# shizukutanaka/Otedama

Hardware: AMD Instinct MI355X
Metric: hashes/sec (whole node) SHA-256d + scrypt at 1/2/4/8 MI355X; p50 share latency (higher is better)
Workload: dtype u32

## Files before the change

### csrc/bindings.cpp

```cpp
#include <pybind11/pybind11.h>
#include <pybind11/stl.h>

#include <array>
#include <atomic>
#include <cstring>
#include <stdexcept>
#include <thread>
#include <tuple>

#include "otedama/aead.h"
#include "otedama/job.h"
#include "otedama/runtime.h"
#include "otedama/trace.h"
#include "otedama/sha256.h"
#include "otedama/sv2_frame.h"
#include "otedama/clock_bounds.h"
#include "otedama/launch_plan.h"
#include "otedama/search_launch.h"
#include "otedama/share_job.h"
#include "otedama/work_queue.h"
#include "otedama/x11.h"

namespace py = pybind11;
using namespace otedama;
// ... 314 lines not shown
  }, py::arg("header"), py::arg("target"), py::arg("start"), py::arg("count"));
  m.def("cpu_scan_method", &cpu_scan_method);
  m.def("_cpu_scan_lanes", [](int lanes, const py::bytes& h, const py::bytes& t, uint32_t start, uint64_t count) {
    std::string hs = need(h, 80, "header"), ts = need(t, 32, "target");
    std::vector<uint32_t> hits;
    {
      py::gil_scoped_release r;
      hits = cpu_scan_sha256d_lanes(lanes, reinterpret_cast<const uint8_t*>(hs.data()),
                                    reinterpret_cast<const uint8_t*>(ts.data()), start, count);
    }
    return hits;
  });
  m.def("merkle_root", [](const py::dict& job, uint64_t en2) {
    auto j = make_job(job); uint8_t root[32];
    merkle_root_from_coinbase(*j, en2, root);
    return to_bytes(root, 32);
  });
  m.def("variant_header", [](const py::dict& job, uint64_t v) {
    auto j = make_job(job);
    uint8_t hdr[80]; uint32_t ver, nt; uint64_t en2;
    j->variant_header(v, hdr, &ver, &nt, &en2);
    return py::make_tuple(to_bytes(hdr, 80), ver, nt, en2);
  });
  m.def("variant_space", [](const py::dict& job) { return make_job(job)->variant_space(); });

  m.def("sha256d_prepare", [](const py::bytes& h, const py::bytes& t) {
    std::string hs = need(h, 80, "header"), ts = need(t, 32, "target");
    Sha256dParams p;
    sha256d_prepare(reinterpret_cast<const uint8_t*>(hs.data()), reinterpret_cast<const uint8_t*>(ts.data()), &p);
    return py::bytes(reinterpret_cast<const char*>(&p), sizeof p);
  });
  m.attr("SHA256D_MAX_K") = kSha256dMaxK;
  {
    py::list ks;
    for (int k = 2; k <= kSha256dMaxK; ++k)
      if (sha256d_k_floor(k) == k) ks.append(k);
    m.attr("SHA256D_K_VALUES") = py::tuple(ks);
  }
  m.def("sha256d_prepare_k", [](const py::list& headers, const py::bytes& t) {
    std::string ts = need(t, 32, "target");
    std::vector<std::string> hs;
    for (auto& h : headers) hs.push_back(need(h.cast<py::bytes>(), 80, "header"));
    std::vector<const uint8_t*> ptrs;
    for (auto& h : hs) ptrs.push_back(reinterpret_cast<const uint8_t*>(h.data()));
    Sha256dParamsK p;
    if (!sha256d_prepare_k(ptrs.data(), (int)ptrs.size(), reinterpret_cast<const uint8_t*>(ts.data()), &p))
      throw std::invalid_argument("need K headers (K in SHA256D_K_VALUES) with identical bytes 64..75");
    return py::bytes(reinterpret_cast<const char*>(&p), sizeof p);
  }, py::arg("headers"), py::arg("target"));
  m.attr("SHA256D_V_GROUP") = kSha256dVGroup;
  m.attr("SHA256D_V2_GROUP") = kSha256dV2Group;
  m.def("sha256d_prepare_v", [](const py::list& headers, const py::bytes& t) {
    std::string ts = need(t, 32, "target");
    std::vector<std::string> hs;
    for (auto& h : headers) hs.push_back(need(h.cast<py::bytes>(), 80, "header"));
    std::vector<const uint8_t*> ptrs;
    for (auto& h : hs) ptrs.push_back(reinterpret_cast<const uint8_t*>(h.data()));
    Sha256dParamsV p;
    std::vector<Sha256dVariant> vars(hs.size());
    if (!sha256d_prepare_v(ptrs.data(), (int)ptrs.size(), reinterpret_cast<const uint8_t*>(ts.data()), &p, vars.data()))
      throw std::invalid_argument("need a positive multiple of 64 headers with identical bytes 64..75");
    return py::make_tuple(py::bytes(reinterpret_cast<const char*>(&p), sizeof p),
                          py::bytes(reinterpret_cast<const char*>(vars.data()), vars.size() * sizeof(Sha256dVariant)));
  }, py::arg("headers"), py::arg("target"));
  m.def("scrypt_prepare", [](const py::bytes& h, const py::bytes& t) {
    std::string hs = need(h, 80, "header"), ts = need(t, 32, "target");
    ScryptParams p;
    scrypt_prepare(reinterpret_cast<const uint8_t*>(hs.data()), reinterpret_cast<const uint8_t*>(ts.data()), &p);
    return py::bytes(reinterpret_cast<const char*>(&p), sizeof p);
  });

  m.def("x11_prepare", [](const py::bytes& h, const py::bytes& t) {
    std::string hs = need(h, 80, "header"), ts = need(t, 32, "target");
    X11Params p;
    x11_prepare(reinterpret_cast<const uint8_t*>(hs.data()), reinterpret_cast<const uint8_t*>(ts.data()), &p);
    return py::bytes(reinterpret_cast<const char*>(&p), sizeof p);
  });

  m.def("trace_push", [](const std::string& name) { trace_push(name.c_str()); });
  m.def("trace_pop", [] { trace_pop(); });
  m.def("trace_mark", [](const std::string& name) { trace_mark(name.c_str()); });
  m.def("gpu_device_count", &gpu_device_count);
  m.def("gpu_arch_name", &gpu_arch_name);
  m.def("gpu_cu_count", &gpu_cu_count);
  m.def("scrypt_scratch_bytes", &scrypt_scratch_bytes);
  m.def("x11_midstage_polls", [] { return x11k::x11_midstage_polls(); });
  m.def("_scrypt_romix_mode", [] {
    bool write_polls = false;
    uint32_t segments = 0;
    scrypt_romix_mode(&write_polls, &segments);
    py::dict d;
    d["write_polls"] = write_polls;
    d["segments"] = segments;
    return d;
  });
  m.def("maps_range_writable", [](const std::string& maps, uint64_t lo, uint64_t hi) {
    return maps_range_writable(maps, uintptr_t(lo), uintptr_t(hi));
  });
  m.def("launch_sha256d", [](const py::bytes& params, uint32_t base, uint64_t count, uintptr_t out, uint32_t cap,
                             int grid, uintptr_t stream) {
    std::string ps = need(params, sizeof(Sha256dParams), "params");
    Sha256dParams p; std::memcpy(&p, ps.data(), sizeof p);
    if (count == 0 || count > (1ull << 32)) throw std::invalid_argument("count must be in [1, 2^32]");
    if (grid <= 0 || out == 0) throw std::invalid_argument("bad grid / out");
    py_launch_sha256d(p, base, count, out, cap, grid, stream);
  }, py::arg("params"), py::arg("base"), py::arg("count"), py::arg("out"), py::arg("cap"), py::arg("grid"),
     py::arg("stream"));
  m.def("launch_sha256d_k", [](const py::bytes& params, uint32_t base, uint64_t count, uintptr_t out, uint32_t cap,
                               int grid, uintptr_t stream) {
    std::string ps = need(params, sizeof(Sha256dParamsK), "params");
    Sha256dParamsK p; std::memcpy(&p, ps.data(), sizeof p);
    if (p.k < 2 || p.k > kSha256dMaxK) throw std::invalid_argument("bad K");
    if (count == 0 || count > (1ull << 32)) throw std::invalid_argument("count must be in [1, 2^32]");
    if (grid <= 0 || out == 0) throw std::invalid_argument("bad grid / out");
    py_launch_sha256d_k(p, base, count, out, cap, grid, stream);
  }, py::arg("params"), py::arg("base"), py::arg("count"), py::arg("out"), py::arg("cap"), py::arg("grid"),
     py::arg("stream"));
  m.def("launch_sha256d_v", [](const py::bytes& params, uintptr_t vars, uint32_t base, uint64_t count, uintptr_t out,
                               uint32_t cap, int grid, uintptr_t stream, bool occupancy8, int block, int chains) {
    std::string ps = need(params, sizeof(Sha256dParamsV), "params");
    Sha256dParamsV p; std::memcpy(&p, ps.data(), sizeof p);
    p.occupancy8 = occupancy8 ? 1u : 0u;
    if (p.groups == 0 || count == 0 || count > (1ull << 32)) throw std::invalid_argument("bad groups / count");
    if (block != 64 && block != 256) throw std::invalid_argument("block must be 64 or 256 threads");
    if (chains < 1 || chains > 4) throw std::invalid_argument("chains must be 1..4");
    if (p.groups % uint32_t(chains) != 0)
      throw std::invalid_argument("chains variants per lane need a multiple of 64 * chains variants");
    if (grid <= 0 || (uint64_t(grid) * uint32_t(block / 64)) % (p.groups / uint32_t(chains)) != 0 || vars == 0 || out == 0)
      throw std::invalid_argument("the wave count must be a multiple of the variant groups; vars/out must be set");
    py_launch_sha256d_v(p, vars, base, count, out, cap, grid, stream, block, chains);
  }, py::arg("params"), py::arg("vars"), py::arg("base"), py::arg("count"), py::arg("out"), py::arg("cap"),
     py::arg("grid"), py::arg("stream"), py::arg("occupancy8") = false, py::arg("block") = 256, py::arg("chains") = 1);
  m.def("launch_scrypt", [](const py::bytes& params, uint32_t base, uint32_t count, uintptr_t xbuf, uintptr_t scratch,
                            int gap, uintptr_t out, uint32_t cap, int grid, uintptr_t stream) {
    std::string ps = need(params, sizeof(ScryptParams), "params");
    ScryptParams p; std::memcpy(&p, ps.data(), sizeof p);
    if (!scrypt_gap_valid(gap))
      throw std::invalid_argument("gap must be 1, 2, 4, SCRYPT_COOP or SCRYPT_LANE_W8");
    if (grid <= 0 || out == 0 || xbuf == 0 || scratch == 0 || count == 0) throw std::invalid_argument("bad launch args");
    py_launch_scrypt(p, base, count, xbuf, scratch, gap, out, cap, grid, stream);
  }, py::arg("params"), py::arg("base"), py::arg("count"), py::arg("xbuf"), py::arg("scratch"), py::arg("gap"),
     py::arg("out"), py::arg("cap"), py::arg("grid"), py::arg("stream"));

  m.def("launch_x11_stage", [](const py::bytes& params, int stage, uint32_t base, uintptr_t H, uint32_t stride,
                               uint32_t n, uintptr_t out, uint32_t cap, uintptr_t stream) {
    std::string ps = need(params, sizeof(X11Params), "params");
    X11Params p; std::memcpy(&p, ps.data(), sizeof p);
    if (stage < 0 || stage >= kX11StageCount) throw std::invalid_argument("stage must be in [0, 11)");
    if (H == 0 || n == 0 || stride < n) throw std::invalid_argument("need H != 0, n > 0, stride >= n");
    py_launch_x11_stage(p, stage, base, H, stride, n, out, cap, stream);
  }, py::arg("params"), py::arg("stage"), py::arg("base"), py::arg("H"), py::arg("stride"), py::arg("n"),
     py::arg("out") = 0, py::arg("cap") = 0, py::arg("stream") = 0);
  m.def("launch_x11", [](const py::bytes& params, uint32_t base, uintptr_t H, uint32_t stride, uint32_t n,
                         uintptr_t out, uint32_t cap, uintptr_t stream) {
    std::string ps = need(params, sizeof(X11Params), "params");
    X11Params p; std::memcpy(&p, ps.data(), sizeof p);
    if (H == 0 || n == 0 || stride < n) throw std::invalid_argument("need H != 0, n > 0, stride >= n");
    py_launch_x11(p, base, H, stride, n, out, cap, stream);
  }, py::arg("params"), py::arg("base"), py::arg("H"), py::arg("stride"), py::arg("n"), py::arg("out") = 0,
     py::arg("cap") = 0, py::arg("stream") = 0);

  m.def("launch_sha256d_digest", [](uintptr_t headers, uint32_t n, uintptr_t out, uintptr_t stream) {
    if (headers == 0 || out == 0 || n == 0) throw std::invalid_argument("need headers != 0, out != 0, n > 0");
    py_launch_sha256d_digest(headers, n, out, stream);
  }, py::arg("headers"), py::arg("n"), py::arg("out"), py::arg("stream") = 0);
  m.def("launch_scrypt_digest", [](uintptr_t headers, uint32_t n, uintptr_t xbuf, uintptr_t scratch, int gap,
                                   uintptr_t out, int grid, uintptr_t stream) {
    if (headers == 0 || out == 0 || xbuf == 0 || scratch == 0 || n == 0 || grid <= 0)
      throw std::invalid_argument("bad launch args");
    if (uint64_t(n) > uint64_t(grid) * 256u) throw std::invalid_argument("n must be at most grid * 256");
    py_launch_scrypt_digest(headers, n, xbuf, scratch, gap, out, grid, stream);
  }, py::arg("headers"), py::arg("n"), py::arg("xbuf"), py::arg("scratch"), py::arg("gap"), py::arg("out"),
     py::arg("grid"), py::arg("stream") = 0);
  m.def("launch_x11_digest", [](uintptr_t headers, uintptr_t H, uint32_t stride, uint32_t n, uintptr_t out,
                                uintptr_t stream) {
    if (headers == 0 || out == 0 || H == 0 || n == 0 || stride < n)
      throw std::invalid_argument("need headers, H, out != 0, n > 0, stride >= n");
    py_launch_x11_digest(headers, H, stride, n, out, stream);
  }, py::arg("headers"), py::arg("H"), py::arg("stride"), py::arg("n"), py::arg("out"), py::arg("stream") = 0);

  m.def("share_job_prepare", [](const py::bytes& coinb1, const py::bytes& coinb2, int en_size,
                                const py::bytes& prev_hash, uint32_t nbits, const std::vector<py::bytes>& branches) {
    std::vector<std::string> bs(branches.begin(), branches.end());
    const ShareJobBlock job = share_job_prepare(coinb1, coinb2, en_size, prev_hash, nbits, bs);
    return py::bytes(reinterpret_cast<const char*>(&job), sizeof job);
  }, py::arg("coinb1"), py::arg("coinb2"), py::arg("en_size"), py::arg("prev_hash"), py::arg("nbits"),
     py::arg("branches"));
  m.def("share_headers_cpu", [](const py::bytes& job_block, const py::bytes& records) {
    std::string js = need(job_block, sizeof(ShareJobBlock), "job_block"), rs = records;
    if (rs.size() % sizeof(ShareRec)) throw std::invalid_argument("records: expected a multiple of 32 bytes");
    ShareJobBlock job;
    std::memcpy(&job, js.data(), sizeof job);
    std::vector<ShareRec> recs(rs.size() / sizeof(ShareRec));
    if (!recs.empty()) std::memcpy(recs.data(), rs.data(), rs.size());
    std::string out(recs.size() * 80, '\0');
    share_headers_cpu(job, recs.data(), recs.size(), reinterpret_cast<uint8_t*>(&out[0]));
    return py::bytes(out);
  }, py::arg("job_block"), py::arg("records"));
  m.attr("SHARE_JOB_BLOCK_SIZE") = sizeof(ShareJobBlock);
  m.def("launch_share_headers", [](uintptr_t job, uintptr_t records, uint32_t n, uintptr_t headers,
                                   uintptr_t stream) {
    if (job == 0 || records == 0 || headers == 0 || n == 0)
      throw std::invalid_argument("need job, records, headers != 0, n > 0");
    if ((job | records | headers) & 15u) throw std::invalid_argument("job, records and headers must be 16-byte aligned");
    py_launch_share_headers(job, records, n, headers, stream);
  }, py::arg("job"), py::arg("records"), py::arg("n"), py::arg("headers"), py::arg("stream") = 0);
  m.def("launch_share_verdict", [](uintptr_t job, uintptr_t records, uintptr_t digests, uintptr_t targets,
                                   uint32_t n_targets, uint32_t n, uintptr_t verdicts, uintptr_t stream) {
    if (job == 0 || records == 0 || digests == 0 || targets == 0 || verdicts == 0 || n == 0 || n_targets == 0)
      throw std::invalid_argument("need job, records, digests, targets, verdicts != 0, n > 0, n_targets > 0");
    if ((job | records | digests | targets) & 15u)
      throw std::invalid_argument("job, records, digests and targets must be 16-byte aligned");
    py_launch_share_verdict(job, records, digests, targets, n_targets, n, verdicts, stream);
  }, py::arg("job"), py::arg("records"), py::arg("digests"), py::arg("targets"), py::arg("n_targets"), py::arg("n"),
     py::arg("verdicts"), py::arg("stream") = 0);

  m.def("share_results_cpu", [](const py::bytes& job_block, const py::bytes& records, const py::bytes& targets) {
    std::string js = need(job_block, sizeof(ShareJobBlock), "job_block"), rs = records, ts = targets;
    if (rs.size() % sizeof(ShareRec)) throw std::invalid_argument("records: expected a multiple of 32 bytes");
    if (ts.empty() || ts.size() % 32) throw std::invalid_argument("targets: expected a non-empty multiple of 32 bytes");
    ShareJobBlock job;
    std::memcpy(&job, js.data(), sizeof job);
    std::vector<ShareRec> recs(rs.size() / sizeof(ShareRec));
    if (!recs.empty()) std::memcpy(recs.data(), rs.data(), rs.size());
    std::vector<ShareResult> out(recs.size());
    share_results_cpu(job, recs.data(), recs.size(), reinterpret_cast<const uint8_t*>(ts.data()), ts.size() / 32,
                      out.data());
    return py::bytes(reinterpret_cast<const char*>(out.data()), out.size() * sizeof(ShareResult));
  }, py::arg("job_block"), py::arg("records"), py::arg("targets"));
  m.attr("SHARE_RESULT_BYTES") = sizeof(ShareResult);
  m.def("launch_share_pack", [](uintptr_t job, uintptr_t records, uintptr_t headers, uintptr_t digests,
                                uintptr_t targets, uint32_t n_targets, uint32_t n, uintptr_t results,
                                uintptr_t stream) {
    if (job == 0 || records == 0 || headers == 0 || digests == 0 || targets == 0 || results == 0 || n == 0 ||
        n_targets == 0)
      throw std::invalid_argument("need job, records, headers, digests, targets, results != 0, n > 0, n_targets > 0");
    if ((job | records | headers | digests | targets | results) & 15u)
      throw std::invalid_argument("job, records, headers, digests, targets and results must be 16-byte aligned");
    py_launch_share_pack(job, records, headers, digests, targets, n_targets, n, results, stream);
  }, py::arg("job"), py::arg("records"), py::arg("headers"), py::arg("digests"), py::arg("targets"),
     py::arg("n_targets"), py::arg("n"), py::arg("results"), py::arg("stream") = 0);

  m.def("share_roots_cpu", [](const py::bytes& job_block, const py::bytes& prefixes) {
    std::string js = need(job_block, sizeof(ShareJobBlock), "job_block"), ps = prefixes;
    if (ps.size() % 16) throw std::invalid_argument("prefixes: expected a multiple of 16 bytes");
    ShareJobBlock job;
    std::memcpy(&job, js.data(), sizeof job);
    std::string out(ps.size() * 2, '\0');
    {
      py::gil_scoped_release r;
      share_roots_cpu(job, reinterpret_cast<const uint8_t*>(ps.data()), ps.size() / 16,
                      reinterpret_cast<uint8_t*>(&out[0]));
    }
    return py::bytes(out);
  }, py::arg("job_block"), py::arg("prefixes"));
  m.def("launch_channel_roots", [](uintptr_t job, uintptr_t prefixes, uint32_t n, uintptr_t roots, uintptr_t stream) {
    if (job == 0 || prefixes == 0 || roots == 0 || n == 0)
      throw std::invalid_argument("need job, prefixes, roots != 0, n > 0");
    if ((job | prefixes | roots) & 15u) throw std::invalid_argument("job, prefixes and roots must be 16-byte aligned");
    py_launch_channel_roots(job, prefixes, n, roots, stream);
  }, py::arg("job"), py::arg("prefixes"), py::arg("n"), py::arg("roots"), py::arg("stream") = 0);

  m.def("merkle_tree_cpu", [](const py::bytes& leaves, uint32_t t, uint32_t n) {
    if (t == 0 || t > kMerkleTreeMaxTrees) throw std::invalid_argument("t must be in 1..65535");
    if (n == 0 || n > kMerkleTreeMaxLeaves) throw std::invalid_argument("n must be in 1..262144");
    std::string ls = need(leaves, size_t(t) * n * 32, "leaves");
    std::string out(size_t(t) * (1 + merkle_tree_depth(n)) * 32, '\0');
    {
      py::gil_scoped_release r;
      merkle_tree_cpu(reinterpret_cast<const uint8_t*>(ls.data()), t, n, reinterpret_cast<uint8_t*>(&out[0]));
    }
    return py::bytes(out);
  }, py::arg("leaves"), py::arg("t"), py::arg("n"));
  m.attr("MERKLE_TREE_MAX_LEAVES") = kMerkleTreeMaxLeaves;
  m.attr("MERKLE_TREE_MAX_TREES") = kMerkleTreeMaxTrees;
  m.def("launch_merkle_tree", [](uintptr_t leaves, uint32_t t, uint32_t n, uintptr_t scratch, uintptr_t out,
                                 uintptr_t stream) {
    if (t == 0 || t > kMerkleTreeMaxTrees || n == 0 || n > kMerkleTreeMaxLeaves)
      throw std::invalid_argument("need t in 1..65535, n in 1..262144");
    if (leaves == 0 || out == 0 || (n > 512 && scratch == 0))
      throw std::invalid_argument("need leaves, out != 0, and scratch != 0 for n > 512");
    if ((leaves | out | scratch) & 15u) throw std::invalid_argument("leaves, scratch and out must be 16-byte aligned");
    py_launch_merkle_tree(leaves, t, n, scratch, out, stream);
  }, py::arg("leaves"), py::arg("t"), py::arg("n"), py::arg("scratch"), py::arg("out"), py::arg("stream") = 0);

  m.def("secp256k1_mul_cpu", [](const py::buffer& rows) {
    const py::buffer_info info = rows.request();
    if (info.ndim != 1 || info.itemsize != 1 || (info.size && info.strides[0] != 1))
      throw std::invalid_argument("rows: expected contiguous bytes");
    const size_t size = size_t(info.size);
    if (size == 0 || size % kSecpRowBytes || size / kSecpRowBytes > kSecpMaxRows)
      throw std::invalid_argument("rows: expected 1..65536 rows of 128 bytes");
    std::string rs(static_cast<const char*>(info.ptr), size);
    const uint32_t n = uint32_t(size / kSecpRowBytes);
    std::string out(size_t(n) * kSecpOutBytes, '\0');
    {
      py::gil_scoped_release r;
      secp256k1_mul_cpu(reinterpret_cast<const uint8_t*>(rs.data()), n, reinterpret_cast<uint8_t*>(&out[0]));
    }
    volatile char* wipe = &rs[0];
    for (size_t i = 0; i < rs.size(); ++i) wipe[i] = 0;
    return py::bytes(out);
  }, py::arg("rows"));
  m.def("ellswift_encode_native", [](const py::bytes& x32, const py::bytes& rand_bytes) -> py::object {
    std::string x = need(x32, 32, "x32"), rnd = rand_bytes;
    uint8_t out[64];
    const int rc = ellswift_encode_cpu(reinterpret_cast<const uint8_t*>(x.data()),
                                       reinterpret_cast<const uint8_t*>(rnd.data()), rnd.size(), out);
    if (rc < 0) throw std::invalid_argument("ellswift: x is not on secp256k1");
    if (rc == 0) return py::none();
    return to_bytes(out, 64);
  }, py::arg("x32"), py::arg("rand_bytes"));
  m.attr("SECP_ROW_BYTES") = kSecpRowBytes;
  m.attr("SECP_OUT_BYTES") = kSecpOutBytes;
  m.attr("SECP_MAX_ROWS") = kSecpMaxRows;
  m.def("launch_secp256k1_mul", [](uintptr_t rows, uint32_t n, uintptr_t out, uintptr_t stream) {
    if (n == 0 || n > kSecpMaxRows) throw std::invalid_argument("need n in 1..65536");
    if (rows == 0 || out == 0) throw std::invalid_argument("need rows, out != 0");
    if ((rows | out) & 15u) throw std::invalid_argument("rows and out must be 16-byte aligned");
    py_launch_secp256k1_mul(rows, n, out, stream);
  }, py::arg("rows"), py::arg("n"), py::arg("out"), py::arg("stream") = 0);

  const auto seal_rows = [](const py::buffer& frames, uint32_t n,
                            void (*fn)(const uint8_t*, size_t, uint32_t, uint8_t*, size_t)) {
    const py::buffer_info info = frames.request();
    if (info.ndim != 1 || info.itemsize != 1 || (info.size && info.strides[0] != 1))
      throw std::invalid_argument("frames: expected contiguous bytes");
    std::string in(static_cast<const char*>(info.ptr), size_t(info.size));
    const auto* ip = reinterpret_cast<const uint8_t*>(in.data());
    std::string out(aead_seal_check(ip, in.size(), n, 0), '\0');
    {
      py::gil_scoped_release r;
      fn(ip, in.size(), n, reinterpret_cast<uint8_t*>(&out[0]), out.size());
    }
    volatile char* wipe = &in[0];
    for (size_t i = 0; i < in.size(); ++i) wipe[i] = 0;
    return py::bytes(out);
  };
  m.def("aead_seal_many_cpu", [seal_rows](const py::buffer& frames, uint32_t n) {
    return seal_rows(frames, n, aead_seal_many_cpu);
  }, py::arg("frames"), py::arg("n"));
  m.def("_aead_seal_rows_host", [seal_rows](const py::buffer& frames, uint32_t n) {
    return seal_rows(frames, n, aead_seal_rows_host);
  }, py::arg("frames"), py::arg("n"));
  m.def("_poly1305_rows_host", [](const py::buffer& rows) {
    const py::buffer_info info = rows.request();
    if (info.ndim != 1 || info.itemsize != 1 || (info.size && info.strides[0] != 1))
      throw std::invalid_argument("rows: expected contiguous bytes");
    const size_t size = size_t(info.size);
    if (size == 0 || size % kPolyRowBytes) throw std::invalid_argument("rows: expected rows of 160 bytes");
    std::string out(size / kPolyRowBytes * 16, '\0');
    poly1305_rows_host(static_cast<const uint8_t*>(info.ptr), uint32_t(size / kPolyRowBytes),
                       reinterpret_cast<uint8_t*>(&out[0]));
    return py::bytes(out);
  }, py::arg("rows"));
  m.attr("SEAL_HEAD_BYTES") = kSealHeadBytes;
  m.attr("SEAL_MAX_PLAIN") = kSealMaxPlain;
  m.attr("SEAL_MAX_FRAMES") = kSealMaxFrames;
  m.attr("POLY_ROW_BYTES") = kPolyRowBytes;
  m.attr("POLY_MAX_MSG") = kPolyMaxMsg;
  m.def("launch_aead_seal", [](uintptr_t frames, uint64_t in_bytes, uint32_t n, uintptr_t out, uint64_t out_bytes,
                               uintptr_t stream) {
    if (n == 0 || n > kSealMaxFrames) throw std::invalid_argument("need n in 1..2^24-1");
    if (frames == 0 || out == 0) throw std::invalid_argument("need frames, out != 0");
    if ((frames | out | in_bytes | out_bytes) & 15u)
      throw std::invalid_argument("frames, out and their sizes must be multiples of 16");
    if (in_bytes < uint64_t(n) * kSealHeadBytes || (in_bytes >> 32) || (out_bytes >> 32))
      throw std::invalid_argument("frames holds n 64-byte heads; both buffers are below 4 GiB");
    py_launch_aead_seal(frames, in_bytes, n, out, out_bytes, stream);
  }, py::arg("frames"), py::arg("in_bytes"), py::arg("n"), py::arg("out"), py::arg("out_bytes"),
     py::arg("stream") = 0);
  m.def("_launch_poly1305_rows", [](uintptr_t rows, uint32_t n, uintptr_t tags, uintptr_t stream) {
    if (n == 0 || n > kSealMaxFrames) throw std::invalid_argument("need n in 1..2^24-1");
    if (rows == 0 || tags == 0) throw std::invalid_argument("need rows, tags != 0");
    if ((rows | tags) & 15u) throw std::invalid_argument("rows and tags must be 16-byte aligned");
    py_launch_poly1305_rows(rows, n, tags, stream);
  }, py::arg("rows"), py::arg("n"), py::arg("tags"), py::arg("stream") = 0);

  py::class_<MinerBase, std::shared_ptr<MinerBase>>(m, "Miner")
      .def("start", &MinerBase::start, py::call_guard<py::gil_scoped_release>())
      .def("stop", &MinerBase::stop, py::call_guard<py::gil_scoped_release>())
      .def("set_job", [](MinerBase& self, py::object job) {
        if (job.is_none()) { py::gil_scoped_release r; self.set_job(nullptr); return; }
        auto j = make_job(job.cast<py::dict>());
        py::gil_scoped_release r;
        self.set_job(j);
      })
      .def("poll", [](MinerBase& self, size_t max) {
        std::vector<ShareRecord> v;
        { py::gil_scoped_release r; v = self.poll(max); }
        return shares_to_list(std::move(v));
      }, py::arg("max") = 256)
      .def("stats", [](MinerBase& self) { return stats_to_dict(self.stats()); })
      .def("share_fd", &MinerBase::share_fd,
           "eventfd that becomes readable when shares are queued (read 8 bytes to reset, then poll())")
      .def_property_readonly("device_id", &MinerBase::device_id);

  py::class_<GpuMiner, MinerBase, std::shared_ptr<GpuMiner>>(m, "GpuMiner")
      .def(py::init<int, std::string, uint64_t, int, size_t, int>(), py::arg("device"), py::arg("device_id"),
           py::arg("batch_nonces") = (1ull << 32), py::arg("grid") = 2048, py::arg("queue_cap") = 1024,
           py::arg("sha_variants") = 128);
  py::class_<CpuMiner, MinerBase, std::shared_ptr<CpuMiner>>(m, "CpuMiner")
      .def(py::init<int, std::string, size_t>(), py::arg("threads"), py::arg("device_id") = "cpu-0",
           py::arg("queue_cap") = 1024);

  m.attr("SHA256D_PARAMS_SIZE") = sizeof(Sha256dParams);
  m.attr("SHA256D_V_PARAMS_SIZE") = sizeof(Sha256dParamsV);
  m.attr("SCRYPT_PARAMS_SIZE") = sizeof(ScryptParams);
}
```

### csrc/cpu/secp256k1.cpp

```cpp
#include "otedama/secp256k1.h"

#include <cstring>
#include <stdexcept>

#include "otedama/secp256k1_curve.h"

namespace otedama {
namespace {

using u128 = unsigned __int128;

struct Fe64 {
  struct fe {
    uint64_t v[4];
  };
  static constexpr uint64_t kFold = 0x1000003D1ull;

  static uint64_t fold(fe& r, uint64_t c) {
    u128 t = u128(c) * kFold;
    for (int i = 0; i < 4; ++i) {
      t += r.v[i];
      r.v[i] = uint64_t(t);
      t >>= 64;
    }
    return uint64_t(t);
  }

  static void reduce_once(fe& r, uint64_t over) {
    fe s = r;
    const uint64_t carry = fold(s, 1);
    const uint64_t m = uint64_t(0) - uint64_t((over | carry) != 0);
    for (int i = 0; i < 4; ++i) r.v[i] = (s.v[i] & m) | (r.v[i] & ~m);
  }

  static fe mul(fe a, fe b) {
    uint64_t r[8] = {};
    for (int i = 0; i < 4; ++i) {
      uint64_t c = 0;
      for (int j = 0; j < 4; ++j) {
        const u128 t = u128(a.v[i]) * b.v[j] + r[i + j] + c;
        r[i + j] = uint64_t(t);
        c = uint64_t(t >> 64);
      }
      r[i + 4] = c;
    }
    fe o;
    u128 t = 0;
    for (int j = 0; j < 4; ++j) {
      t += u128(r[4 + j]) * kFold + r[j];
      o.v[j] = uint64_t(t);
      t >>= 64;
    }
    uint64_t c = fold(o, uint64_t(t));
    c = fold(o, c);
    reduce_once(o, 0);
    return o;
  }
  static fe sqr(fe a) { return mul(a, a); }

  static fe add(fe a, fe b) {
    fe s;
    u128 t = 0;
    for (int i = 0; i < 4; ++i) {
      t += u128(a.v[i]) + b.v[i];
      s.v[i] = uint64_t(t);
      t >>= 64;
    }
    reduce_once(s, uint64_t(t));
    return s;
  }

  static fe sub(fe a, fe b) {
    fe d;
    uint64_t borrow = 0;
    for (int i = 0; i < 4; ++i) {
      const u128 t = u128(a.v[i]) - b.v[i] - borrow;
      d.v[i] = uint64_t(t);
      borrow = uint64_t(t >> 64) & 1u;
    }
    fe e;
    uint64_t bw = 0;
    for (int i = 0; i < 4; ++i) {
      const u128 t = u128(d.v[i]) - (i == 0 ? kFold : 0) - bw;
      e.v[i] = uint64_t(t);
      bw = uint64_t(t >> 64) & 1u;
    }
    const uint64_t m = uint64_t(0) - borrow;
    for (int i = 0; i < 4; ++i) d.v[i] = (e.v[i] & m) | (d.v[i] & ~m);
    return d;
  }

  static fe select(bool c, fe a, fe b) {
    const uint64_t m = uint64_t(0) - uint64_t(c);
    fe r;
    for (int i = 0; i < 4; ++i) r.v[i] = (a.v[i] & m) | (b.v[i] & ~m);
    return r;
  }
  static bool is_zero(fe a) { return (a.v[0] | a.v[1] | a.v[2] | a.v[3]) == 0; }
  static bool odd(fe a) { return (a.v[0] & 1u) != 0; }
  static fe small(uint32_t v) { return fe{{v, 0, 0, 0}}; }
  static fe from_words(const uint32_t w[8]) {
    fe r;
    for (int i = 0; i < 4; ++i) r.v[i] = uint64_t(w[2 * i]) | (uint64_t(w[2 * i + 1]) << 32);
    reduce_once(r, 0);
    return r;
  }
  static void to_words(fe a, uint32_t w[8]) {
    for (int i = 0; i < 4; ++i) {
      w[2 * i] = uint32_t(a.v[i]);
      w[2 * i + 1] = uint32_t(a.v[i] >> 32);
    }
  }
};

using C = secp::Curve<Fe64>;
using fe = Fe64::fe;

void load_be(const uint8_t* b, uint32_t w[8]) {
  for (int i = 0; i < 8; ++i) {
    const uint8_t* p = b + 4 * (7 - i);
    w[i] = (uint32_t(p[0]) << 24) | (uint32_t(p[1]) << 16) | (uint32_t(p[2]) << 8) | p[3];
  }
}

void store_be(const uint32_t w[8], uint8_t* b) {
  for (int i = 0; i < 8; ++i) {
    uint8_t* p = b + 4 * (7 - i);
    p[0] = uint8_t(w[i] >> 24);
    p[1] = uint8_t(w[i] >> 16);
    p[2] = uint8_t(w[i] >> 8);
    p[3] = uint8_t(w[i]);
  }
}

fe neg(fe a) { return Fe64::sub(Fe64::small(0), a); }

bool xswiftec_inv(fe x, fe u, unsigned which, fe& t) {
  const uint32_t cw[8] = OTD_SECP_C, hw[8] = OTD_SECP_HALF;
  const fe c = C::constant(cw), half = C::constant(hw);
  const fe g = C::curve_rhs(u);
  fe v, s;
  if ((which & 2) == 0) {
    if (C::is_x(Fe64::sub(neg(x), u))) return false;
    v = x;
    const fe den = Fe64::add(Fe64::add(Fe64::sqr(u), Fe64::mul(u, v)), Fe64::sqr(v));
    if (Fe64::is_zero(den)) return false;
    s = Fe64::mul(neg(g), C::inv(den));
  } else {
    s = Fe64::sub(x, u);
    if (Fe64::is_zero(s)) return false;
    const fe g4 = Fe64::add(Fe64::add(g, g), Fe64::add(g, g));
    const fe su2 = Fe64::mul(s, Fe64::sqr(u));
    const fe inner = Fe64::add(g4, Fe64::add(Fe64::add(su2, su2), su2));
    fe r;
    if (!C::sqrt(Fe64::mul(neg(s), inner), r)) return false;
    if ((which & 1) && Fe64::is_zero(r)) return false;
    v = Fe64::mul(Fe64::sub(Fe64::mul(r, C::inv(s)), u), half);
  }
  fe w;
  if (!C::sqrt(s, w) || Fe64::is_zero(w)) return false;
  const unsigned k = which & 5;
  const fe one = Fe64::small(1);
  const fe cc = (k == 0 || k == 4) ? Fe64::sub(one, c) : Fe64::add(one, c);
  const fe body = Fe64::mul(w, Fe64::add(Fe64::mul(Fe64::mul(u, cc), half), v));
  t = (k == 0 || k == 5) ? neg(body) : body;
  return true;
}

}

void secp256k1_mul_cpu(const uint8_t* rows, uint32_t n, uint8_t* out) {
  if (n == 0 || n > kSecpMaxRows) throw std::invalid_argument("secp256k1_mul_cpu: n must be in 1..65536");
  for (uint32_t i = 0; i < n; ++i) {
    const uint8_t* in = rows + size_t(i) * kSecpRowBytes;
    uint8_t* o = out + size_t(i) * kSecpOutBytes;
    uint32_t k[8], pa[8], pb[8], x[8], parity = 0;
    load_be(in, k);
    load_be(in + 32, pa);
    load_be(in + 64, pb);
    const uint32_t status = C::row(k, pa, pb, in[96], x, parity);
    std::memset(o, 0, kSecpOutBytes);
    store_be(x, o);
    o[32] = uint8_t(status);
    o[33] = uint8_t(parity);
    volatile uint32_t* wipe = k;
    for (int j = 0; j < 8; ++j) wipe[j] = 0;
  }
}

int ellswift_encode_cpu(const uint8_t x32[32], const uint8_t* rnd, size_t rnd_len, uint8_t out[64]) {
  const uint32_t pw[8] = OTD_SECP_P;
  uint32_t xw[8];
  load_be(x32, xw);
  if (secp::words_ge(xw, pw)) return -1;
  const fe x = Fe64::from_words(xw);
  if (!C::is_x(x)) return -1;
  for (size_t at = 0; at + 33 <= rnd_len; at += 33) {
    uint32_t uw[8], tw[8];
    load_be(rnd + at, uw);
    const fe u = Fe64::from_words(uw);
    if (Fe64::is_zero(u)) continue;
    fe t;
    if (!xswiftec_inv(x, u, rnd[at + 32] & 7u, t) || Fe64::is_zero(t)) continue;
    Fe64::to_words(u, uw);
    Fe64::to_words(t, tw);
    store_be(uw, out);
    store_be(tw, out + 32);
    return 1;
  }
  return 0;
}

}
```

### csrc/include/otedama/secp256k1.h

```cpp
#pragma once
#include <cstddef>
#include <cstdint>

namespace otedama {

constexpr uint32_t kSecpRowBytes = 128;
constexpr uint32_t kSecpOutBytes = 48;
constexpr uint32_t kSecpMaxRows = 65536;

constexpr uint32_t kSecpKindG = 0, kSecpKindXOnly = 1, kSecpKindEllSwift = 2;
constexpr uint32_t kSecpOk = 0, kSecpBadScalar = 1, kSecpBadPoint = 2, kSecpBadKind = 3;

void secp256k1_mul_cpu(const uint8_t* rows, uint32_t n, uint8_t* out);

int ellswift_encode_cpu(const uint8_t x[32], const uint8_t* rnd, size_t rnd_len, uint8_t out[64]);

}
```

### csrc/include/otedama/secp256k1_curve.h

```cpp
#pragma once
#include <cstdint>

#include "otedama/secp256k1.h"

#if defined(__HIPCC__)
#define OTD_SECP_FN __host__ __device__ inline
#define OTD_SECP_ROLLED _Pragma("unroll 1")
#else
#define OTD_SECP_FN inline
#define OTD_SECP_ROLLED
#endif

namespace otedama {
namespace secp {

#define OTD_SECP_N {0xD0364141u, 0xBFD25E8Cu, 0xAF48A03Bu, 0xBAAEDCE6u, 0xFFFFFFFEu, 0xFFFFFFFFu, 0xFFFFFFFFu, 0xFFFFFFFFu}
#define OTD_SECP_P {0xFFFFFC2Fu, 0xFFFFFFFEu, 0xFFFFFFFFu, 0xFFFFFFFFu, 0xFFFFFFFFu, 0xFFFFFFFFu, 0xFFFFFFFFu, 0xFFFFFFFFu}
#define OTD_SECP_GX {0x16F81798u, 0x59F2815Bu, 0x2DCE28D9u, 0x029BFCDBu, 0xCE870B07u, 0x55A06295u, 0xF9DCBBACu, 0x79BE667Eu}
#define OTD_SECP_GY {0xFB10D4B8u, 0x9C47D08Fu, 0xA6855419u, 0xFD17B448u, 0x0E1108A8u, 0x5DA4FBFCu, 0x26A3C465u, 0x483ADA77u}
#define OTD_SECP_C {0x1CD5F852u, 0x7D8D27AEu, 0xDA14ECD4u, 0xC61F6D15u, 0xA797962Cu, 0x233770C2u, 0x3507F1DFu, 0x0A2D2BA9u}
#define OTD_SECP_HALF {0x7FFFFE18u, 0xFFFFFFFFu, 0xFFFFFFFFu, 0xFFFFFFFFu, 0xFFFFFFFFu, 0xFFFFFFFFu, 0xFFFFFFFFu, 0x7FFFFFFFu}

OTD_SECP_FN bool words_ge(const uint32_t a[8], const uint32_t b[8]) {
  uint32_t borrow = 0;
#pragma unroll
  for (int i = 0; i < 8; ++i) {
    const uint64_t d = uint64_t(a[i]) - b[i] - borrow;
    borrow = uint32_t(d >> 63);
  }
  return borrow == 0;
}

OTD_SECP_FN bool words_zero(const uint32_t a[8]) {
  uint32_t o = 0;
#pragma unroll
  for (int i = 0; i < 8; ++i) o |= a[i];
  return o == 0;
}

template <class F>
struct Curve {
  using fe = typename F::fe;

  struct Jac {
    fe x, y, z;
  };

  static OTD_SECP_FN fe constant(const uint32_t (&w)[8]) { return F::from_words(w); }

  static OTD_SECP_FN fe sqrn(fe a, int n) {
    OTD_SECP_ROLLED
    for (int i = 0; i < n; ++i) a = F::sqr(a);
    return a;
  }

  static OTD_SECP_FN fe pow_chain(fe a, bool root) {
    const fe x2 = F::mul(F::sqr(a), a);
    const fe x3 = F::mul(F::sqr(x2), a);
    const fe x6 = F::mul(sqrn(x3, 3), x3);
    const fe x9 = F::mul(sqrn(x6, 3), x3);
    const fe x11 = F::mul(sqrn(x9, 2), x2);
    const fe x22 = F::mul(sqrn(x11, 11), x11);
    const fe x44 = F::mul(sqrn(x22, 22), x22);
    const fe x88 = F::mul(sqrn(x44, 44), x44);
    const fe x176 = F::mul(sqrn(x88, 88), x88);
    const fe x220 = F::mul(sqrn(x176, 44), x44);
    const fe x223 = F::mul(sqrn(x220, 3), x3);
    fe t = F::mul(sqrn(x223, 23), x22);
    if (root) {
      t = F::mul(sqrn(t, 6), x2);
      return sqrn(t, 2);
    }
    t = F::mul(sqrn(t, 5), a);
    t = F::mul(sqrn(t, 3), x2);
    return F::mul(sqrn(t, 2), a);
  }

  static OTD_SECP_FN fe inv(fe a) { return pow_chain(a, false); }

  static OTD_SECP_FN bool sqrt(fe a, fe& r) {
    r = pow_chain(a, true);
    return F::is_zero(F::sub(F::sqr(r), a));
  }

  static OTD_SECP_FN fe curve_rhs(fe x) { return F::add(F::mul(F::sqr(x), x), F::small(7)); }

  static OTD_SECP_FN bool is_x(fe x) {
    fe r;
    return sqrt(curve_rhs(x), r);
  }

  static OTD_SECP_FN bool lift_even(fe x, fe& y) {
    fe r;
    const bool on = sqrt(curve_rhs(x), r);
    y = F::select(F::odd(r), F::sub(F::small(0), r), r);
    return on;
  }

  static OTD_SECP_FN fe xswiftec(fe u, fe t) {
    const uint32_t cw[8] = OTD_SECP_C, hw[8] = OTD_SECP_HALF;
    const fe half = constant(hw);
    if (F::is_zero(u)) u = F::small(1);
    if (F::is_zero(t)) t = F::small(1);
    const fe g = curve_rhs(u);
    if (F::is_zero(F::add(g, F::sqr(t)))) t = F::add(t, t);
    const fe X = F::mul(F::sub(g, F::sqr(t)), inv(F::add(t, t)));
    const fe Y = F::mul(F::add(X, t), inv(F::mul(constant(cw), u)));
    const fe y2 = F::sqr(Y);
    const fe y4 = F::add(y2, y2);
    const fe x1 = F::add(u, F::add(y4, y4));
    if (is_x(x1)) return x1;
    const fe xy = F::mul(X, inv(Y));
    const fe x2 = F::mul(F::sub(F::sub(F::small(0), xy), u), half);
    if (is_x(x2)) return x2;
    return F::mul(F::sub(xy, u), half);
  }

  static OTD_SECP_FN Jac jselect(bool c, const Jac& a, const Jac& b) {
    Jac r;
    r.x = F::select(c, a.x, b.x);
    r.y = F::select(c, a.y, b.y);
    r.z = F::select(c, a.z, b.z);
    return r;
  }

  static OTD_SECP_FN Jac jdouble(const Jac& p) {
    const fe ysq = F::sqr(p.y);
    fe s = F::mul(p.x, ysq);
    s = F::add(s, s);
    s = F::add(s, s);
    const fe xx = F::sqr(p.x);
    const fe m = F::add(F::add(xx, xx), xx);
    Jac r;
    r.x = F::sub(F::sub(F::sqr(m), s), s);
    fe y4 = F::sqr(ysq);
    y4 = F::add(y4, y4);
    y4 = F::add(y4, y4);
    y4 = F::add(y4, y4);
    r.y = F::sub(F::mul(m, F::sub(s, r.x)), y4);
    const fe yz = F::mul(p.y, p.z);
    r.z = F::add(yz, yz);
    return r;
  }

  static OTD_SECP_FN Jac jadd_affine(const Jac& p, fe x2, fe y2) {
    const fe z1z1 = F::sqr(p.z);
    const fe u2 = F::mul(x2, z1z1);
    const fe s2 = F::mul(F::mul(y2, p.z), z1z1);
    const fe h = F::sub(u2, p.x);
    const fe r = F::sub(s2, p.y);
    const fe hh = F::sqr(h);
    const fe hhh = F::mul(h, hh);
    const fe v = F::mul(p.x, hh);
    Jac o;
    o.x = F::sub(F::sub(F::sub(F::sqr(r), hhh), v), v);
    o.y = F::sub(F::mul(r, F::sub(v, o.x)), F::mul(p.y, hhh));
    o.z = F::mul(p.z, h);
    return o;
  }

  static OTD_SECP_FN void mul(const uint32_t k[8], fe px, fe py, fe& rx, fe& ry) {
    uint32_t kk[8];
#pragma unroll
    for (int i = 0; i < 8; ++i) kk[i] = k[i];
    Jac base, acc;
    base.x = px;
    base.y = py;
    base.z = F::small(1);
    acc.x = F::small(0);
    acc.y = F::small(1);
    acc.z = F::small(0);
    bool inf = true;
    OTD_SECP_ROLLED
    for (int i = 0; i < 256; ++i) {
      const bool bit = (kk[7] >> 31) != 0;
#pragma unroll
      for (int j = 7; j > 0; --j) kk[j] = (kk[j] << 1) | (kk[j - 1] >> 31);
      kk[0] <<= 1;
      const Jac d = jdouble(acc);
      const Jac s = jselect(inf, base, jadd_affine(d, px, py));
      acc = jselect(bit, s, d);
      inf = inf & !bit;
    }
    const fe zi = inv(acc.z);
    const fe zi2 = F::sqr(zi);
    rx = F::mul(acc.x, zi2);
    ry = F::mul(acc.y, F::mul(zi2, zi));
  }

  static OTD_SECP_FN uint32_t row(const uint32_t k[8], const uint32_t pa[8], const uint32_t pb[8], uint32_t kind,
                                  uint32_t x[8], uint32_t& parity) {
    const uint32_t nw[8] = OTD_SECP_N, pw[8] = OTD_SECP_P, gx[8] = OTD_SECP_GX, gy[8] = OTD_SECP_GY;
    uint32_t status = kSecpOk;
    fe px = constant(gx), py = constant(gy);
    if (kind > kSecpKindEllSwift) {
      status = kSecpBadKind;
    } else if (words_zero(k) || words_ge(k, nw)) {
      status = kSecpBadScalar;
    } else if (kind == kSecpKindXOnly) {
      fe y;
      const fe xx = F::from_words(pa);
      if (words_ge(pa, pw) || !lift_even(xx, y)) {
        status = kSecpBadPoint;
      } else {
        px = xx;
        py = y;
      }
    } else if (kind == kSecpKindEllSwift) {
      px = xswiftec(F::from_words(pa), F::from_words(pb));
      lift_even(px, py);
    }
    uint32_t kk[8];
#pragma unroll
    for (int i = 0; i < 8; ++i) kk[i] = status == kSecpOk ? k[i] : (i == 0 ? 1u : 0u);
    if (status != kSecpOk) {
      px = constant(gx);
      py = constant(gy);
    }
    fe rx, ry;
    mul(kk, px, py, rx, ry);
    uint32_t xw[8];
    F::to_words(rx, xw);
    const uint32_t keep = status == kSecpOk ? 0xFFFFFFFFu : 0u;
#pragma unroll
    for (int i = 0; i < 8; ++i) x[i] = xw[i] & keep;
    parity = (F::odd(ry) ? 1u : 0u) & keep;
    return status;
  }
};

}
}
```

Baseline: 19.31 billion.

## Use GLV endomorphism to halve secp256k1 scalar multiplication loop

The scalar is split with the GLV decomposition into two roughly 128-bit halves, so the double-and-add ladder runs 128 iterations instead of 256 and uses a shared Shamir-style table built from P, beta*P and their sum. Points are kept in a common Z coordinate so the table entries can still be added as affine points. The main cost removed is about half of the point doublings and additions per row. In exchange it adds the split arithmetic, a select tree per step and a new CPU binding, and the precomputed sum can hit degenerate cases.

```diff
diff --git a/csrc/bindings.cpp b/csrc/bindings.cpp
--- a/csrc/bindings.cpp
+++ b/csrc/bindings.cpp
@@ -640,6 +640,12 @@
     for (size_t i = 0; i < rs.size(); ++i) wipe[i] = 0;
     return py::bytes(out);
   }, py::arg("rows"));
+  m.def("secp256k1_glv_split", [](const py::bytes& k32) {
+    const std::string k = need(k32, 32, "k32");
+    uint8_t out[34];
+    secp256k1_glv_split_cpu(reinterpret_cast<const uint8_t*>(k.data()), out);
+    return py::make_tuple(to_bytes(out, 16), out[32] != 0, to_bytes(out + 16, 16), out[33] != 0);
+  }, py::arg("k32"));
   m.def("ellswift_encode_native", [](const py::bytes& x32, const py::bytes& rand_bytes) -> py::object {
     std::string x = need(x32, 32, "x32"), rnd = rand_bytes;
     uint8_t out[64];
diff --git a/csrc/cpu/secp256k1.cpp b/csrc/cpu/secp256k1.cpp
--- a/csrc/cpu/secp256k1.cpp
+++ b/csrc/cpu/secp256k1.cpp
@@ -188,6 +188,21 @@
   }
 }
 
+void secp256k1_glv_split_cpu(const uint8_t k[32], uint8_t out[34]) {
+  uint32_t kw[8], m1[4], m2[4];
+  bool neg1, neg2;
+  load_be(k, kw);
+  secp::glv_split(kw, m1, neg1, m2, neg2);
+  for (int i = 0; i < 4; ++i) {
+    for (int b = 0; b < 4; ++b) {
+      out[4 * (3 - i) + b] = uint8_t(m1[i] >> (24 - 8 * b));
+      out[16 + 4 * (3 - i) + b] = uint8_t(m2[i] >> (24 - 8 * b));
+    }
+  }
+  out[32] = uint8_t(neg1);
+  out[33] = uint8_t(neg2);
+}
+
 int ellswift_encode_cpu(const uint8_t x32[32], const uint8_t* rnd, size_t rnd_len, uint8_t out[64]) {
   const uint32_t pw[8] = OTD_SECP_P;
   uint32_t xw[8];
diff --git a/csrc/include/otedama/secp256k1.h b/csrc/include/otedama/secp256k1.h
--- a/csrc/include/otedama/secp256k1.h
+++ b/csrc/include/otedama/secp256k1.h
@@ -13,6 +13,8 @@
 
 void secp256k1_mul_cpu(const uint8_t* rows, uint32_t n, uint8_t* out);
 
+void secp256k1_glv_split_cpu(const uint8_t k[32], uint8_t out[34]);
+
 int ellswift_encode_cpu(const uint8_t x[32], const uint8_t* rnd, size_t rnd_len, uint8_t out[64]);
 
 }
diff --git a/csrc/include/otedama/secp256k1_curve.h b/csrc/include/otedama/secp256k1_curve.h
--- a/csrc/include/otedama/secp256k1_curve.h
+++ b/csrc/include/otedama/secp256k1_curve.h
@@ -20,6 +20,13 @@
 #define OTD_SECP_GY {0xFB10D4B8u, 0x9C47D08Fu, 0xA6855419u, 0xFD17B448u, 0x0E1108A8u, 0x5DA4FBFCu, 0x26A3C465u, 0x483ADA77u}
 #define OTD_SECP_C {0x1CD5F852u, 0x7D8D27AEu, 0xDA14ECD4u, 0xC61F6D15u, 0xA797962Cu, 0x233770C2u, 0x3507F1DFu, 0x0A2D2BA9u}
 #define OTD_SECP_HALF {0x7FFFFE18u, 0xFFFFFFFFu, 0xFFFFFFFFu, 0xFFFFFFFFu, 0xFFFFFFFFu, 0xFFFFFFFFu, 0xFFFFFFFFu, 0x7FFFFFFFu}
+#define OTD_SECP_BETA {0x719501EEu, 0xC1396C28u, 0x12F58995u, 0x9CF04975u, 0xAC3434E9u, 0x6E64479Eu, 0x657C0710u, 0x7AE96A2Bu}
+#define OTD_SECP_GLV_G1 {0x45DBB031u, 0xE893209Au, 0x71E8CA7Fu, 0x3DAA8A14u, 0x9284EB15u, 0xE86C90E4u, 0xA7D46BCDu, 0x3086D221u}
+#define OTD_SECP_GLV_G2 {0x8AC47F71u, 0x1571B4AEu, 0x9DF506C6u, 0x221208ACu, 0x0ABFE4C4u, 0x6F547FA9u, 0x010E8828u, 0xE4437ED6u}
+#define OTD_SECP_GLV_A1 {0x9284EB15u, 0xE86C90E4u, 0xA7D46BCDu, 0x3086D221u, 0x00000000u}
+#define OTD_SECP_GLV_A2 {0x9D44CFD8u, 0x57C1108Du, 0xA8E2F3F6u, 0x14CA50F7u, 0x00000001u}
+#define OTD_SECP_GLV_MB1 {0x0ABFE4C3u, 0x6F547FA9u, 0x010E8828u, 0xE4437ED6u, 0x00000000u}
+#define OTD_SECP_GLV_B2 {0x9284EB15u, 0xE86C90E4u, 0xA7D46BCDu, 0x3086D221u, 0x00000000u}
 
 OTD_SECP_FN bool words_ge(const uint32_t a[8], const uint32_t b[8]) {
   uint32_t borrow = 0;
@@ -36,6 +43,84 @@
 #pragma unroll
   for (int i = 0; i < 8; ++i) o |= a[i];
   return o == 0;
+}
+
+OTD_SECP_FN void glv_quotient(const uint32_t k[8], const uint32_t (&g)[8], uint32_t c[4]) {
+  uint32_t r[16];
+#pragma unroll
+  for (int i = 0; i < 16; ++i) r[i] = 0;
+#pragma unroll
+  for (int i = 0; i < 8; ++i) {
+    uint32_t carry = 0;
+#pragma unroll
+    for (int j = 0; j < 8; ++j) {
+      const uint64_t t = uint64_t(k[i]) * g[j] + r[i + j] + carry;
+      r[i + j] = uint32_t(t);
+      carry = uint32_t(t >> 32);
+    }
+    r[i + 8] = carry;
+  }
+  uint64_t t = r[11] >> 31;
+#pragma unroll
+  for (int i = 0; i < 4; ++i) {
+    t += r[12 + i];
+    c[i] = uint32_t(t);
+    t >>= 32;
+  }
+}
+
+OTD_SECP_FN void glv_mul_low(const uint32_t a[4], const uint32_t (&b)[5], uint32_t w[5]) {
+#pragma unroll
+  for (int i = 0; i < 5; ++i) w[i] = 0;
+#pragma unroll
+  for (int i = 0; i < 4; ++i) {
+    uint32_t carry = 0;
+#pragma unroll
+    for (int j = 0; j < 5 - i; ++j) {
+      const uint64_t t = uint64_t(a[i]) * b[j] + w[i + j] + carry;
+      w[i + j] = uint32_t(t);
+      carry = uint32_t(t >> 32);
+    }
+  }
+}
+
+OTD_SECP_FN void glv_sub(const uint32_t a[5], const uint32_t b[5], uint32_t d[5]) {
+  uint32_t borrow = 0;
+#pragma unroll
+  for (int i = 0; i < 5; ++i) {
+    const uint64_t t = uint64_t(a[i]) - b[i] - borrow;
+    d[i] = uint32_t(t);
+    borrow = uint32_t(t >> 63);
+  }
+}
+
+OTD_SECP_FN bool glv_abs(const uint32_t w[5], uint32_t m[4]) {
+  const uint32_t neg = w[4] >> 31, mask = 0u - neg;
+  uint64_t t = neg;
+#pragma unroll
+  for (int i = 0; i < 4; ++i) {
+    t += w[i] ^ mask;
+    m[i] = uint32_t(t);
+    t >>= 32;
+  }
+  return neg != 0;
+}
+
+OTD_SECP_FN void glv_split(const uint32_t k[8], uint32_t m1[4], bool& neg1, uint32_t m2[4], bool& neg2) {
+  const uint32_t g1[8] = OTD_SECP_GLV_G1, g2[8] = OTD_SECP_GLV_G2;
+  const uint32_t a1[5] = OTD_SECP_GLV_A1, a2[5] = OTD_SECP_GLV_A2, mb1[5] = OTD_SECP_GLV_MB1, b2[5] = OTD_SECP_GLV_B2;
+  uint32_t c1[4], c2[4], s[5], t[5], w[5];
+  glv_quotient(k, g1, c1);
+  glv_quotient(k, g2, c2);
+  glv_mul_low(c1, a1, s);
+  glv_sub(k, s, w);
+  glv_mul_low(c2, a2, s);
+  glv_sub(w, s, t);
+  neg1 = glv_abs(t, m1);
+  glv_mul_low(c1, mb1, s);
+  glv_mul_low(c2, b2, t);
+  glv_sub(s, t, w);
+  neg2 = glv_abs(w, m2);
 }
 
 template <class F>
@@ -160,29 +245,48 @@
   }
 
   static OTD_SECP_FN void mul(const uint32_t k[8], fe px, fe py, fe& rx, fe& ry) {
-    uint32_t kk[8];
-#pragma unroll
-    for (int i = 0; i < 8; ++i) kk[i] = k[i];
-    Jac base, acc;
-    base.x = px;
-    base.y = py;
-    base.z = F::small(1);
+    const uint32_t bw[8] = OTD_SECP_BETA;
+    uint32_t u[4], v[4];
+    bool neg1, neg2;
+    glv_split(k, u, neg1, v, neg2);
+    const fe one = F::small(1);
+    const fe ny = F::sub(F::small(0), py);
+    Jac p1;
+    p1.x = px;
+    p1.y = F::select(neg1, ny, py);
+    p1.z = one;
+    const Jac s = jadd_affine(p1, F::mul(constant(bw), px), F::select(neg2, ny, py));
+    const fe zz = F::sqr(s.z);
+    const fe x1 = F::mul(px, zz);
+    const fe x2 = F::mul(constant(bw), x1);
+    const fe yy = F::mul(py, F::mul(zz, s.z));
+    const fe nyy = F::sub(F::small(0), yy);
+    const fe y1 = F::select(neg1, nyy, yy), y2 = F::select(neg2, nyy, yy);
+    Jac acc;
     acc.x = F::small(0);
-    acc.y = F::small(1);
+    acc.y = one;
     acc.z = F::small(0);
     bool inf = true;
     OTD_SECP_ROLLED
-    for (int i = 0; i < 256; ++i) {
-      const bool bit = (kk[7] >> 31) != 0;
-#pragma unroll
-      for (int j = 7; j > 0; --j) kk[j] = (kk[j] << 1) | (kk[j - 1] >> 31);
-      kk[0] <<= 1;
+    for (int i = 0; i < 128; ++i) {
+      const bool b1 = (u[3] >> 31) != 0, b2 = (v[3] >> 31) != 0;
+#pragma unroll
+      for (int j = 3; j > 0; --j) {
+        u[j] = (u[j] << 1) | (u[j - 1] >> 31);
+        v[j] = (v[j] << 1) | (v[j - 1] >> 31);
+      }
+      u[0] <<= 1;
+      v[0] <<= 1;
+      Jac t;
+      t.x = F::select(b1, F::select(b2, s.x, x1), x2);
+      t.y = F::select(b1, F::select(b2, s.y, y1), y2);
+      t.z = one;
+      const bool any = b1 | b2;
       const Jac d = jdouble(acc);
-      const Jac s = jselect(inf, base, jadd_affine(d, px, py));
-      acc = jselect(bit, s, d);
-      inf = inf & !bit;
-    }
-    const fe zi = inv(acc.z);
+      acc = jselect(any, jselect(inf, t, jadd_affine(d, t.x, t.y)), d);
+      inf = inf & !any;
+    }
+    const fe zi = inv(F::mul(acc.z, s.z));
     const fe zi2 = F::sqr(zi);
     rx = F::mul(acc.x, zi2);
     ry = F::mul(acc.y, F::mul(zi2, zi));
```

New measurement: 19.34 billion (median of 6 runs). About the same (+0.2%).
